# wells-wood-research/timed-design

Measured on AMD Instinct MI355X. Metric: residue_frames_per_sec, higher is better.
Workload: dtype f32

## Files before the change

timed-design_amd/csrc/common.h:

```cpp
#pragma once
#include <hip/hip_runtime.h>
#include <stdint.h>
#include <string>
#include <vector>

#include "../../include/timed_hip.h"

enum : int {
    OP_INPUT = 0, OP_CONV3D, OP_DENSE, OP_BN, OP_ACT, OP_MAXPOOL, OP_AVGPOOL, OP_GAP, OP_GMP,
    OP_FLATTEN, OP_CONCAT, OP_ADD, OP_IDENTITY
};
enum : int { ACT_LINEAR = 0, ACT_RELU, ACT_ELU, ACT_SOFTMAX, ACT_SIGMOID, ACT_TANH, ACT_LEAKY };

void th_set_error(const char* fmt, ...);
#define TH_FAIL(code, ...)          \
    do {                            \
        th_set_error(__VA_ARGS__);  \
        return (code);              \
    } while (0)
#define HIP_TRY(expr)                                                                            \
    do {                                                                                         \
        hipError_t _e = (expr);                                                                  \
        if (_e != hipSuccess) {                                                                  \
            th_set_error("%s failed: %s (%s:%d)", #expr, hipGetErrorString(_e), __FILE__, __LINE__); \
            return TH_EHIP;                                                                      \
        }                                                                                        \
    } while (0)

struct ThKnobs {
    int winograd = 1;
    int wino_split = 1;
    int wfused = 1;
    int wf_split = 1;
    int lanes = 1, lane_lag = 1;
    int guard = 1;
    int first_wino = 1;
    int first_split = 1;
    int conv_gl = 1;
    int dense_gemm = 1;
    int first_int = 1;
    int first_zb = 0;
    int first_dbg = 0;
    int no_pool_first = 0;
    int no_tail_fuse = 0;
    int conv_nogeo = 0, n16_nogeo = 0, conv_noxc = 0, conv_notail = 0, conv_nozmajor = 0, conv_nocompact = 0, conv_nopw = 0;
    int conv_bmode = 0;
    int conv_dbg = 0, conv_ldspad = 0, n16_resident = 0;
    int pw_nopipe = 0, pw_noepi = 0, pw_dbg = 0;
    int wf_resident = 0, wf_dbg = 0, wf_noblk = 0;
    long long wino_piece = 0;
    int wino_dbg = 0, wino_var = 3, wino_b3var = 0, wino_nomid = 0;
    std::string nondefault;
};
void th_knobs_read(ThKnobs* k);
inline const ThKnobs& th_knobs_of(const ThKnobs* k) { static const ThKnobs dflt; return k ? *k : dflt; }

hipError_t th_malloc_retry_impl(void** p, size_t bytes);
template <class T> inline hipError_t th_malloc_retry(T** p, size_t bytes) { return th_malloc_retry_impl(reinterpret_cast<void**>(p), bytes); }

int th_usable_cpus();

struct TView {
    float* p = nullptr;
    int D = 1, H = 1, W = 1, C = 0;
    int cs = 0;
    int coff = 0;
    int64_t fs = 0;
    int blk = 0;
    int V() const { return D * H * W; }
};

#define TH_MAX_POST 4
enum : int { POP_ACT = 1, POP_AFFINE = 2 };
struct PostOps {
    int n = 0;
    int type[TH_MAX_POST] = {0, 0, 0, 0};
    int act[TH_MAX_POST] = {0, 0, 0, 0};
    float alpha[TH_MAX_POST] = {0, 0, 0, 0};
    const float* scale[TH_MAX_POST] = {nullptr, nullptr, nullptr, nullptr};
    const float* shift[TH_MAX_POST] = {nullptr, nullptr, nullptr, nullptr};
    int monotone = 0;
};
struct PreOp {
    const float* scale = nullptr;
    const float* shift = nullptr;
    int act = ACT_LINEAR;
    float alpha = 0.f;
};

struct ConvGeom {
    int kd, kh, kw, sd, sh, sw, dd, dh, dw;
    int pz, py, px;
};
int launch_convert_frames(hipStream_t s, const void* src, int dtype, int64_t n, int V, int C, TView dst);
int launch_conv3d_direct(hipStream_t s, int64_t n, TView in, TView out, ConvGeom g, const float* w, const float* bias,
                         PreOp pre, PostOps post);
int launch_pool3d(hipStream_t s, int64_t n, TView in, TView out, ConvGeom g, int is_max);
int launch_eltwise(hipStream_t s, int64_t n, TView in, TView out, PostOps ops);
int launch_global_pool(hipStream_t s, int64_t n, TView in, TView out, int is_max);
int launch_dense(hipStream_t s, int64_t n, TView in, TView out, const float* w, const float* bias, PostOps post);
inline bool conv_gl_wanted(int knob, const ConvGeom& g, int Vo) { return knob == 2 || (knob == 1 && (g.sd > 1 || g.sh > 1 || g.sw > 1 || Vo <= 64)); }
bool conv_gl_ok(int Cin, int Cout, int in_cs, int in_coff, int64_t in_fs);
size_t conv_gl_wpk_floats(const ConvGeom& g, int Cin, int Cout);
double conv_gl_exec_flops(const ConvGeom& g, int Cin, int Cout, int Vo);
std::string conv_gl_label(int Cout);
void conv_gl_pack_weights(const ConvGeom& g, int Cin, int Cout, const float* w, float* dst);
int launch_conv_gl(hipStream_t s, int64_t n, TView in, TView out, ConvGeom g, int Cin, int Cout, const float* wpk, const float* bias, PreOp pre, PostOps post);
bool dense_gemm_ok(int F, int O, int64_t xfs);
int launch_dense_gemm(hipStream_t s, int64_t n, TView in, TView out, const float* w, const float* bias, PostOps post);
int launch_softmax(hipStream_t s, int64_t n, TView in, TView out);
int launch_gap_softmax(hipStream_t s, int64_t n, TView in, TView logits, TView probs);
int launch_tail_dense(hipStream_t s, int64_t n, TView in, PostOps pre, TView pooled, TView logits, TView probs, const float* w,
                      const float* bias, PostOps post, int softmax);
int launch_copy(hipStream_t s, int64_t n, TView in, TView out);
int launch_add(hipStream_t s, int64_t n, TView a, TView b, TView out);
int launch_synth_frames(hipStream_t s, float* d, int64_t n, int side, int channels, int atoms, uint64_t seed);

struct ConvMfmaPlan {
    int cfg = -1;
    int CI = 0, CS = 0;
    int BN = 0;
    int nnb = 0;
    int nchunks = 0;
    int pool = 0;
    int Dc = 0, Hc = 0, Wc = 0;
    int FB = 1, ZB = 0, nzb = 1;
    int Zp = 0, Hp = 0, Wp = 0;
    int rows_pf = 0;
    int bres = 0;
    int ncu = 0;
    size_t lds_bytes = 0;
    size_t tab_off = 0;
    size_t wpk_floats = 0;
    double exec_flops = 0;
    int first_wino = 0;
    double own_flops = 0;
    int geo = 0;
    const ThKnobs* knobs = nullptr;
    std::string label;
};
bool conv_mfma_plan(const TView& in, const TView& out_conv, const ConvGeom& g, int Cin, int Cout, int pool,
                    const ThKnobs& kn, ConvMfmaPlan* plan);
bool conv_mfma_plan_tail(const TView& in, const TView& out_conv, const ConvGeom& g, int Cin, int Cout, int pool,
                         const ConvMfmaPlan& main, const ThKnobs& kn, ConvMfmaPlan* tail, int* cout_main);
void conv_mfma_pack_weights(const ConvMfmaPlan& p, const ConvGeom& g, int Cin, int Cout, const float* w_keras,
                            float* dst);
int launch_conv_mfma(hipStream_t s, int64_t n, const ConvMfmaPlan& p, TView in, TView out, ConvGeom g, int Cin,
                     int Cout, const float* wpk, const float* bias, PreOp pre, PostOps post);

struct ConvWinoPlan {
    int P = 9;
    int Cin = 0, Cout = 0, Coutp = 0, ncb = 0;
    int Cinp = 0;
    size_t wpk_floats = 0;
    int64_t v_fpf = 0, m_fpf = 0;
    double gemm_flops = 0;
    double exec_flops = 0;
    int split = 0;
    int narrow = 0;
    const ThKnobs* knobs = nullptr;
    std::string label;
};
bool conv_wino_plan(const TView& in, const TView& out_conv, const ConvGeom& g, int Cin, int Cout, int scheme, int split, const ThKnobs& kn,
                    ConvWinoPlan* plan);
void conv_wino_pack_weights(const ConvWinoPlan& p, const float* w_keras, float* dst);
int launch_wino_in(hipStream_t s, int64_t n, const ConvWinoPlan& p, TView in, float* V, PreOp pre);
int launch_wino_gemm(hipStream_t s, int64_t n, const ConvWinoPlan& p, const float* V, float* M, const float* wpk);
int launch_wino_out(hipStream_t s, int64_t n, const ConvWinoPlan& p, const float* M, TView out, const float* bias, PostOps post, bool gap = false);
int launch_wino_mid(hipStream_t s, int64_t n, const ConvWinoPlan& p, const float* M, float* V_next, const float* bias, PostOps post);

struct ConvWfPlan {
    int geo = -1;
    int pool = 0;
    int Cin = 0, Cout = 0, ncb = 0, nchunks = 0;
    size_t wpk_floats = 0, lds_bytes = 0;
    double own_flops = 0;
    double exec_flops = 0;
    int ncu = 0;
    const ThKnobs* knobs = nullptr;
    std::string label;
};
bool conv_wf_plan(const TView& in, const TView& out_conv, const ConvGeom& g, int Cin, int Cout, int pool, const ThKnobs& kn, ConvWfPlan* plan);
bool conv_wf_view_ok(const TView& in);
int conv_wf_pre_kind(const PreOp& pre);
std::string conv_wf_label(const ConvWfPlan& p, const PreOp& pre);
void conv_wf_pack_weights(const ConvWfPlan& p, const float* w_keras, float* dst);
int launch_conv_wf(hipStream_t s, int64_t n, const ConvWfPlan& p, TView in, TView out, const float* wpk, const float* bias, PreOp pre,
                   PostOps post);

struct ConvWfsPlan {
    int geo = -1, pool = 0;
    int Cin = 0, Cout = 0, nkh = 0, ncp = 0;
    size_t wpk_floats = 0, lds_bytes = 0;
    double own_flops = 0, exec_flops = 0;
    int ncu = 0;
    const ThKnobs* knobs = nullptr;
    std::string label;
};
bool conv_wfs_plan(const ConvWfPlan& base, const TView& in, const PreOp& pre, const ThKnobs& kn, ConvWfsPlan* plan);
void conv_wfs_pack_weights(const ConvWfsPlan& p, const float* w_keras, float* dst);
int launch_conv_wfs(hipStream_t s, int64_t n, const ConvWfsPlan& p, TView in, TView out, const float* wpk, const float* bias, PostOps post);

int launch_sparse_expand(hipStream_t s, int64_t n, const uint32_t* bits, const uint64_t* vidx, const float* values, float* out, int E, int W);

std::string conv_first_label(const ConvMfmaPlan& p, int Cin, const PostOps& post);
bool conv_first_plan(int Din, int Hin, int Win, int Cin, const TView& out_conv, const ConvGeom& g, int Cout, int pool,
                     const ThKnobs& kn, ConvMfmaPlan* plan);
void conv_first_pack_weights(int Cin, int Cout, const float* w_keras, float* dst);
void conv_first_w_pack_weights(int Cin, int Cout, const float* w_keras, float* dst);
int launch_conv_first(hipStream_t s, int64_t n, const ConvMfmaPlan& p, const void* frames, int dtype, int Din, int Hin,
                      int Win, int Cin, TView out, ConvGeom g, int Cout, const float* wpk, const float* bias, PostOps post);
bool conv_first_b3_ok(const ConvMfmaPlan& p, int Din, int Hin, int Win, int Cin, int Cout, const ConvGeom& g, const PostOps& post);
size_t conv_first_b3_wpk_floats();
double conv_first_b3_exec_flops();
std::string conv_first_b3_label(int nnb);
void conv_first_b3_pack_weights(int Cin, int Cout, const float* w_keras, float* dst);
int launch_conv_first_b3(hipStream_t s, int64_t n, const ConvMfmaPlan& p, const void* frames, int dtype, int Cin, TView out, int Cout,
                         const float* wpk, const float* bias, PostOps post);

bool conv_first5_ok(int Din, int Hin, int Win, int Cin, int Cout, const ConvGeom& g, int pool, const ThKnobs& kn);
size_t conv_first5_wpk_floats();
double conv_first5_exec_flops();
std::string conv_first5_label();
void conv_first5_pack_weights(int Cin, int Cout, const float* w_keras, float* dst);
int launch_conv_first5(hipStream_t s, int64_t n, const ThKnobs* knobs, int ncu, const void* frames, int dtype, int Cin, TView out, int Cout,
                       const float* wpk, const float* bias, PostOps post);

bool conv_pw_plan(const TView& in, const TView& out_conv, const ConvGeom& g, int Cin, int Cout, int pool, const ThKnobs& kn, ConvMfmaPlan* plan);
void conv_pw_pack_weights(const ConvMfmaPlan& p, int Cin, int Cout, const float* w_keras, float* dst);
std::string conv_pw_label(const ConvMfmaPlan& p, bool out_blk, const PostOps& post);
int launch_conv_pw(hipStream_t s, int64_t n, const ConvMfmaPlan& p, TView in, TView out, int Cin, int Cout, const float* wpk,
                   const float* bias, PreOp pre, PostOps post);

int sampler_run(int device, const double* h_probs, int64_t n_res, int n_cls, int64_t n_samples, double temperature,
                int rng_mode, uint64_t seed, uint64_t rng_offset, const double* h_uniforms, int32_t* h_idx, double* h_r_out,
                const char* cat_letters, char* h_letters, double* h_q_out);
```

timed-design_amd/csrc/conv_wino.hip:

```cpp
#include "common.h"
#include "device_math.h"
#include "wino_tables.h"

#include <algorithm>
#include <cstdlib>
#include <cstring>
#include <thread>
#include <vector>

typedef float f32x16 __attribute__((ext_vector_type(16)));

namespace {

constexpr int kZ = WINO_N;
constexpr int kNF = 64;
constexpr int kKC = 32;
constexpr int kCB = 128;

template <int R, int C>
__device__ __forceinline__ void wino_apply(const float (&T)[R][C], const float (&in)[C], float (&out)[R]) {
#pragma unroll
    for (int r = 0; r < R; ++r) {
        float acc = 0.f;
        bool first = true;
// ... 318 lines not shown
                if (ph + 1 < kSlots * kZ) {
                    const int ns = (ph + 1) / kZ, nz = (ph + 1) % kZ;
                    af[cur ^ 1][0] = *reinterpret_cast<const float4*>(lds + aoff[ns] + (nz * kNF) * kKC);
                    af[cur ^ 1][1] = *reinterpret_cast<const float4*>(lds + aoff[ns] + (nz * kNF + 32) * kKC);
                }
                if (VAR == 1) __builtin_amdgcn_sched_barrier(0);
                const float av0[4] = {af[cur][0].x, af[cur][0].y, af[cur][0].z, af[cur][0].w};
                const float av1[4] = {af[cur][1].x, af[cur][1].y, af[cur][1].z, af[cur][1].w};
#pragma unroll
                for (int dz = 0; dz < 3; ++dz) {
                    if (!wino_tap_ok(zi, dz)) continue;
                    const int zo = zi - dz + 1;
                    const float4 b4 = bw[s & 1][dz];
                    const float bv[4] = {b4.x, b4.y, b4.z, b4.w};
#pragma unroll
                    for (int t = 0; t < 4; ++t) {
                        acc[zo][0] = __builtin_amdgcn_mfma_f32_32x32x2f32(av0[t], bv[t], acc[zo][0], 0, 0, 0);
                        acc[zo][1] = __builtin_amdgcn_mfma_f32_32x32x2f32(av1[t], bv[t], acc[zo][1], 0, 0, 0);
                    }
                }
                if (VAR == 1) __builtin_amdgcn_sched_barrier(0);
            }
        }
    }
    if (!active) return;
    float* mbase = a.M + ((int64_t)p * a.Ns + (int64_t)fb * kNF) * a.Coutp + cb * kCB + wave * 32 + j;
    const int64_t mz = (int64_t)a.npos * a.Ns * a.Coutp;
    if (a.dbg & 2) {
        float sum = 0.f;
#pragma unroll
        for (int z = 0; z < kZ; ++z)
#pragma unroll
            for (int rt = 0; rt < 2; ++rt)
#pragma unroll
                for (int r = 0; r < 16; ++r) sum += acc[z][rt][r];
        if (sum == 12345.678f) mbase[0] = sum;
        return;
    }
    if (VAR == 3) {
        __syncthreads();
        float* T = lds + wave * (32 * 36);
        const int rr = lane >> 3, c4 = (lane & 7) * 4;
        float* mb = a.M + ((int64_t)p * a.Ns + (int64_t)fb * kNF) * a.Coutp + cb * kCB + wave * 32 + c4;
#pragma unroll
        for (int z = 0; z < kZ; ++z)
#pragma unroll
            for (int rt = 0; rt < 2; ++rt) {
#pragma unroll
                for (int r = 0; r < 16; ++r) T[((r & 3) + 8 * (r >> 2) + 4 * h) * 36 + j] = acc[z][rt][r];
#pragma unroll
                for (int k = 0; k < 4; ++k) {
                    const int row = rr + 8 * k;
                    *reinterpret_cast<float4*>(mb + z * mz + (int64_t)(rt * 32 + row) * a.Coutp) = *reinterpret_cast<const float4*>(T + row * 36 + c4);
                }
            }
        return;
    }
#pragma unroll
    for (int z = 0; z < kZ; ++z)
#pragma unroll
        for (int rt = 0; rt < 2; ++rt)
#pragma unroll
            for (int r = 0; r < 16; ++r) {
                const int row = rt * 32 + (r & 3) + 8 * (r >> 2) + 4 * h;
                if (VAR == 2) __builtin_nontemporal_store(acc[z][rt][r], mbase + z * mz + (int64_t)row * a.Coutp);
                else mbase[z * mz + (int64_t)row * a.Coutp] = acc[z][rt][r];
            }
}


typedef __bf16 bf16x8 __attribute__((ext_vector_type(8)));
typedef __bf16 bf16x2 __attribute__((ext_vector_type(2)));
typedef float f32x2v __attribute__((ext_vector_type(2)));
typedef unsigned u32x4v __attribute__((ext_vector_type(4)));

__device__ __forceinline__ unsigned wino_pk_bf16(float lo, float hi) {
    return __builtin_bit_cast(unsigned, __builtin_convertvector((f32x2v){lo, hi}, bf16x2));
}
__device__ __forceinline__ float wino_bf16_lo(unsigned w) { return __builtin_bit_cast(float, w << 16); }
__device__ __forceinline__ float wino_bf16_hi(unsigned w) { return __builtin_bit_cast(float, w & 0xffff0000u); }

constexpr int kB3Slab = kZ * kNF * kKC * 2;

template <int VAR>
__global__ void __launch_bounds__(256, 2) k_wino_gemm_b3(const WinoGemmArgs a) {
    __shared__ __attribute__((aligned(16))) unsigned char lds[3 * kB3Slab];
    const unsigned xcd = blockIdx.x & 7u, slot = blockIdx.x >> 3;
    const unsigned L = xcd * a.per_xcd + slot;
    if (slot >= a.per_xcd || L >= a.total) return;
    const unsigned cb = L % (unsigned)a.ncb;
    const unsigned fb = (L / (unsigned)a.ncb) % (unsigned)a.nfb;
    const unsigned p = L / (unsigned)(a.ncb * a.nfb);
    const int tid = threadIdx.x, lane = tid & 63;
    const int wave = __builtin_amdgcn_readfirstlane(tid >> 6);
    const int j = lane & 31, h = lane >> 5;
    const int nchunks = a.Cin / kKC;
    const bool active = (int)(cb * kCB) + wave * 32 < a.Cout;
    const int S = nchunks * 6;
    const uint4* wq = reinterpret_cast<const uint4*>(a.U) + ((size_t)((p * a.ncb + cb) * 4 + wave) * S * 3) * 64 + lane;
    const float* vbase = a.V + ((int64_t)p * a.Ns + (int64_t)fb * kNF) * a.Cin;
    const int64_t zstride = (int64_t)a.npos * a.Ns * a.Cin;

    f32x16 acc[kZ][2];
#pragma unroll
    for (int z = 0; z < kZ; ++z)
#pragma unroll
        for (int rt = 0; rt < 2; ++rt)
#pragma unroll
            for (int r = 0; r < 16; ++r) acc[z][rt][r] = 0.f;

    uint4 bw[2][3];
#pragma unroll
    for (int pc = 0; pc < 3; ++pc) bw[0][pc] = wq[pc * 64];
    const int r0 = 8 * wave + (lane >> 3), g4 = lane & 7;
    __amdgpu_buffer_rsrc_t vrsrc[kZ];
#pragma unroll
    for (int z = 0; z < kZ; ++z) vrsrc[z] = __builtin_amdgcn_make_buffer_rsrc(const_cast<float*>(vbase + z * zstride), 0, 0xffffffffu, 0x00020000);
    const unsigned goff = (unsigned)(r0 * a.Cin + 4 * g4) * 4u;
    const unsigned rstride32_b = (unsigned)(32 * a.Cin * 4);
    unsigned char* const sdst = lds + r0 * 64 + (((g4 >> 1) ^ ((r0 >> 2) & 3)) << 4) + ((g4 & 1) << 3);
    const unsigned char* aptr[2];
#pragma unroll
    for (int ks = 0; ks < 2; ++ks) aptr[ks] = lds + j * 64 + (((2 * ks + h) ^ ((j >> 2) & 3)) << 4);

    for (int ch = 0; ch < nchunks; ++ch) {
        __syncthreads();
        {
            float4 x[10];
#pragma unroll
            for (int i = 0; i < 10; ++i)
                x[i] = (a.dbg & 1) ? make_float4(1.f, 2.f, 3.f, 4.f) :
                       __builtin_bit_cast(float4, __builtin_amdgcn_raw_buffer_load_b128(vrsrc[i >> 1], goff, (i & 1) * rstride32_b + ch * (kKC * 4), 0));
            __builtin_amdgcn_sched_barrier(0);
#pragma unroll
            for (int i = 0; i < 10; ++i) {
                const unsigned h01 = wino_pk_bf16(x[i].x, x[i].y), h23 = wino_pk_bf16(x[i].z, x[i].w);
                const float rx = x[i].x - wino_bf16_lo(h01), ry = x[i].y - wino_bf16_hi(h01);
                const float rz = x[i].z - wino_bf16_lo(h23), rw = x[i].w - wino_bf16_hi(h23);
                const unsigned m01 = wino_pk_bf16(rx, ry), m23 = wino_pk_bf16(rz, rw);
                const float sx = rx - wino_bf16_lo(m01), sy = ry - wino_bf16_hi(m01);
                const float sz = rz - wino_bf16_lo(m23), sw = rw - wino_bf16_hi(m23);
                const unsigned l01 = wino_pk_bf16(sx, sy), l23 = wino_pk_bf16(sz, sw);
                *reinterpret_cast<uint2*>(sdst + i * 2048) = make_uint2(h01, h23);
                *reinterpret_cast<uint2*>(sdst + i * 2048 + kB3Slab) = make_uint2(m01, m23);
                *reinterpret_cast<uint2*>(sdst + i * 2048 + 2 * kB3Slab) = make_uint2(l01, l23);
            }
        }
        __syncthreads();
        if (!active) continue;
#pragma unroll
        for (int st = 0; st < 6; ++st) {
            const int ks = st / 3, dz = st % 3, cur = st & 1;
            {
                const int sg = ch * 6 + st;
                const int nx = sg + 1 < S ? sg + 1 : sg;
                if (a.dbg & 4) {
#pragma unroll
                    for (int pc = 0; pc < 3; ++pc) bw[cur ^ 1][pc] = bw[cur][pc];
                } else
#pragma unroll
                for (int pc = 0; pc < 3; ++pc) bw[cur ^ 1][pc] = wq[(size_t)(nx * 3 + pc) * 64];
            }
            bf16x8 bf[3];
#pragma unroll
            for (int pc = 0; pc < 3; ++pc) bf[pc] = __builtin_bit_cast(bf16x8, bw[cur][pc]);
            const int nzi = 5 - (dz != 1), z0 = dz == 2 ? 1 : 0;
            bf16x8 af[2][2][3];
            auto read_a = [&](int set, int zi) {
#pragma unroll
// ... 100 lines not shown
        for (int q = 0; q < 4; ++q) {
            hw[q] = wino_pk_bf16(v[2 * q], v[2 * q + 1]);
            const float r0 = v[2 * q] - wino_bf16_lo(hw[q]), r1 = v[2 * q + 1] - wino_bf16_hi(hw[q]);
            mw[q] = wino_pk_bf16(r0, r1);
            const float s0 = r0 - wino_bf16_lo(mw[q]), s1 = r1 - wino_bf16_hi(mw[q]);
            lw[q] = wino_pk_bf16(s0, s1);
        }
        f[0] = __builtin_bit_cast(bf16x8, make_uint4(hw[0], hw[1], hw[2], hw[3]));
        f[1] = __builtin_bit_cast(bf16x8, make_uint4(mw[0], mw[1], mw[2], mw[3]));
        f[2] = __builtin_bit_cast(bf16x8, make_uint4(lw[0], lw[1], lw[2], lw[3]));
    };

    float4 xs[3][4];
    auto load_step = [&](float4 (&x)[4], int step_ch, int zi) {
        load_plane(x, step_ch < nchunks ? step_ch : nchunks - 1, zi);
    };
    load_step(xs[0], 0, 0);
    load_step(xs[1], 0, 1);
    for (int ch0 = 0; ch0 < nchunks; ch0 += 3) {
#pragma unroll
        for (int cc = 0; cc < 3; ++cc) {
            const int ch = ch0 + cc;
            if (ch >= nchunks) break;
            uint4 bw[2][3][3];
#pragma unroll
            for (int ks = 0; ks < 2; ++ks)
#pragma unroll
                for (int dz = 0; dz < 3; ++dz)
#pragma unroll
                    for (int pc = 0; pc < 3; ++pc) bw[ks][dz][pc] = wq[(size_t)(((ch * 2 + ks) * 3 + dz) * 3 + pc) * 64];
#pragma unroll
            for (int zi = 0; zi < kZ; ++zi) {
                const int t = cc * kZ + zi;
                float4 fr[4];
                transpose(xs[t % 3], fr);
                {
                    const int t2 = t + 2, c2 = ch0 + t2 / kZ, z2 = t2 % kZ;
                    load_step(xs[t2 % 3], c2, z2);
                }
                bf16x8 af[2][3];
                split8(fr[0], fr[1], af[0]);
                split8(fr[2], fr[3], af[1]);
                constexpr int PA[6] = {2, 0, 1, 1, 0, 0}, PB[6] = {0, 2, 1, 0, 1, 0};
#pragma unroll
                for (int q = 0; q < 6; ++q)
#pragma unroll
                    for (int ks = 0; ks < 2; ++ks)
#pragma unroll
                        for (int dz = 0; dz < 3; ++dz) {
                            if (!wino_tap_ok(zi, dz)) continue;
                            acc[zi - dz + 1] = __builtin_amdgcn_mfma_f32_32x32x16_bf16(af[ks][PA[q]], __builtin_bit_cast(bf16x8, bw[ks][dz][PB[q]]),
                                                                                       acc[zi - dz + 1], 0, 0, 0);
                        }
                __builtin_amdgcn_sched_barrier(0);
            }
        }
    }
    float* mb = a.M + ((int64_t)p * a.Ns + (int64_t)fb * 32) * a.Coutp + j;
    const int64_t mz = (int64_t)a.npos * a.Ns * a.Coutp;
#pragma unroll
    for (int z = 0; z < kZ; ++z)
#pragma unroll
        for (int r = 0; r < 16; ++r) mb[z * mz + (int64_t)((r & 3) + 8 * (r >> 2) + 4 * h) * a.Coutp] = acc[z][r];
}

}

bool conv_wino_plan(const TView& in, const TView& out, const ConvGeom& g, int Cin, int Cout, int scheme, int split, const ThKnobs& kn, ConvWinoPlan* p) {
    if (g.kd != 3 || g.kh != 3 || g.kw != 3 || g.sd != 1 || g.sh != 1 || g.sw != 1 || g.dd != 1 || g.dh != 1 || g.dw != 1) return false;
    if (g.pz != 1 || g.py != 1 || g.px != 1) return false;
    if (in.D != kZ || in.H != kZ || in.W != kZ || out.D != kZ || out.H != kZ || out.W != kZ) return false;
    const bool narrow = split && Cout <= 32 && Cin >= 128;
    if (Cin < kKC || (Cout < 64 && !narrow)) return false;
    if (scheme != 9 && scheme != 7) return false;
    const int kPos = scheme * scheme;
    p->P = scheme;
    p->Cin = Cin; p->Cout = Cout;
    p->Cinp = (Cin + kKC - 1) / kKC * kKC;
    const int Cinp = p->Cinp;
    p->narrow = narrow ? 1 : 0;
    p->Coutp = narrow ? 32 : (Cout + kCB - 1) / kCB * kCB;
    p->ncb = narrow ? 1 : p->Coutp / kCB;
    p->split = split ? 1 : 0;
    p->knobs = &kn;
    p->wpk_floats = (size_t)kPos * 3 * Cinp * p->Coutp * (p->split ? 3 : 2) / 2;
    p->v_fpf = (int64_t)kZ * kPos * Cinp;
    p->m_fpf = (int64_t)kZ * kPos * p->Coutp;
    p->gemm_flops = 2.0 * kPos * 13 * Cin * (double)Cout;
    p->exec_flops = 2.0 * kPos * 13 * Cinp * (double)((Cout + 31) / 32 * 32);
    p->label = std::string("conv_wino<") + (scheme == 9 ? "F(3,3)+F(2,3)" : "F(5,3)") + " in-plane, z direct; gemm " + (narrow ? "32f x 32" : "64f x " + std::to_string(kCB)) + "c, K" + std::to_string(Cinp) + (Cinp != Cin ? " (" + std::to_string(Cin) + " real)" : "") +
               (p->split ? "; bf16x3 split operands, 6 products, fp32 accumulate" : "") + ">";
    return true;
}

static inline uint16_t wino_bf16_rne(float f) {
    uint32_t u;
    std::memcpy(&u, &f, 4);
    if ((u & 0x7f800000u) == 0x7f800000u) return (uint16_t)(u >> 16);
    u += 0x7fffu + ((u >> 16) & 1u);
    return (uint16_t)(u >> 16);
}
static inline double wino_bf16_val(uint16_t b) {
    const uint32_t u = (uint32_t)b << 16;
    float f;
    std::memcpy(&f, &u, 4);
    return (double)f;
}
static inline void wino_split3(double x, uint16_t (&pc)[3]) {
    pc[0] = wino_bf16_rne((float)x);
    const double r1 = x - wino_bf16_val(pc[0]);
    pc[1] = wino_bf16_rne((float)r1);
    const double r2 = r1 - wino_bf16_val(pc[1]);
    pc[2] = wino_bf16_rne((float)r2);
}

void conv_wino_pack_weights(const ConvWinoPlan& p, const float* w, float* dst) {
    const int Cin = p.Cin, Cinp = p.Cinp, Cout = p.Cout, S = Cinp / 8, ncb = p.ncb, kP = p.P;
    auto G = [kP](int a, int j) { return kP == 9 ? kWinoG9[a][j] : kWinoG7[a][j]; };
    std::memset(dst, 0, p.wpk_floats * sizeof(float));
    auto work = [&](int ci_lo, int ci_hi) {
        std::vector<double> t((size_t)kP * 3 * Cout), u((size_t)Cout);
        for (int ci = ci_lo; ci < ci_hi; ++ci) {
            const int s = ci / 8, hh = (ci % 8) / 4, tt = ci % 4;
            for (int dz = 0; dz < 3; ++dz) {
                for (int a = 0; a < kP; ++a)
                    for (int k = 0; k < 3; ++k) {
                        double* tr = &t[((size_t)a * 3 + k) * Cout];
                        std::fill(tr, tr + Cout, 0.0);
                        for (int jj = 0; jj < 3; ++jj) {
                            const double g = G(a, jj);
                            if (g == 0.0) continue;
                            const float* wr = w + ((((size_t)dz * 3 + jj) * 3 + k) * Cin + ci) * Cout;
                            for (int co = 0; co < Cout; ++co) tr[co] += g * (double)wr[co];
                        }
                    }
                for (int a = 0; a < kP; ++a)
                    for (int b = 0; b < kP; ++b) {
                        std::fill(u.begin(), u.end(), 0.0);
                        for (int k = 0; k < 3; ++k) {
                            const double g = G(b, k);
                            if (g == 0.0) continue;
                            const double* tr = &t[((size_t)a * 3 + k) * Cout];
                            for (int co = 0; co < Cout; ++co) u[co] += g * tr[co];
                        }
                        const int pos = a * kP + b;
                        if (p.narrow) {
                            uint16_t* d16 = reinterpret_cast<uint16_t*>(dst);
                            const int chunk = ci / kKC, h16 = (ci % kKC) / 16, ks = (ci % 16) / 8, e = ci % 8, nch = Cinp / kKC;
                            for (int co = 0; co < Cout; ++co) {
                                uint16_t pc[3];
                                wino_split3(u[co], pc);
                                const size_t frag = ((size_t)(pos * nch + chunk) * 2 + ks) * 3 + dz;
                                for (int q = 0; q < 3; ++q) d16[((frag * 3 + q) * 64 + (h16 * 32 + co)) * 8 + e] = pc[q];
                            }
                            continue;
                        }
                        if (p.split) {
                            uint16_t* d16 = reinterpret_cast<uint16_t*>(dst);
                            const int chunk = ci / kKC, ks = (ci % kKC) / 16, h8 = (ci % 16) / 8, e = ci % 8, nsteps = (Cinp / kKC) * 6;
                            for (int co = 0; co < Cout; ++co) {
                                const int cb = co / kCB, wv = (co % kCB) / 32, j = co % 32;
                                uint16_t pc[3];
                                wino_split3(u[co], pc);
                                const size_t step = (size_t)((pos * ncb + cb) * 4 + wv) * nsteps + (size_t)(chunk * 2 + ks) * 3 + dz;
                                for (int q = 0; q < 3; ++q) d16[((step * 3 + q) * 64 + (h8 * 32 + j)) * 8 + e] = pc[q];
                            }
                            continue;
                        }
                        for (int co = 0; co < Cout; ++co) {
                            const int cb = co / kCB, wv = (co % kCB) / 32, j = co % 32;
                            dst[((((size_t)(pos * ncb + cb) * 4 + wv) * S + s) * 3 + dz) * 256 + (hh * 32 + j) * 4 + tt] = (float)u[co];
                        }
                    }
            }
        }
    };
    const int nt = std::max(1, std::min({th_usable_cpus(), 32, Cin / 8}));
    if (nt == 1) { work(0, Cin); return; }
    std::vector<std::thread> th;
    for (int k = 0; k < nt; ++k) th.emplace_back(work, (int)((int64_t)Cin * k / nt), (int)((int64_t)Cin * (k + 1) / nt));
    for (auto& x : th) x.join();
}

static int64_t wino_piece(const ConvWinoPlan& p, int64_t n, int64_t Ns, int64_t fs, int width) {
    const int64_t lim = (1ll << 31) - 1;
    if (Ns * width > lim) return 0;
    const int64_t forced = th_knobs_of(p.knobs).wino_piece;
    const int64_t piece = std::max<int64_t>(1, std::min<int64_t>(n, lim / std::max<int64_t>(fs, 1)));
    return forced > 0 ? std::min(piece, forced) : piece;
}

int launch_wino_in(hipStream_t s, int64_t n, const ConvWinoPlan& p, TView in, float* V, PreOp pre) {
    if (n <= 0) return TH_OK;
    const int64_t Ns = (n + kNF - 1) / kNF * kNF;
    const int64_t piece = wino_piece(p, n, Ns, in.fs, p.Cinp);
    if (!piece) TH_FAIL(TH_EUNSUP, "conv_wino: %lld frames per launch exceed the 32-bit offsets of the transform kernels", (long long)n);
    const bool has_pre = pre.scale || pre.act != ACT_LINEAR;
    for (int64_t f0 = 0; f0 < n; f0 += piece) {
        const int64_t cnt = std::min(piece, n - f0);
        WinoInArgs ia;
        ia.in = in.p + f0 * in.fs; ia.in_fs = in.fs; ia.in_cs = in.cs; ia.in_coff = in.coff; ia.Cin = p.Cinp; ia.Creal = p.Cin; ia.pre = pre;
        ia.V = V + f0 * p.Cinp; ia.Ns = Ns; ia.n = cnt;
        const dim3 grid((unsigned)((cnt * p.Cinp + 255) / 256));
        if (p.P == 9) {
            if (has_pre) hipLaunchKernelGGL((k_wino_in<true, 9>), grid, dim3(256), 0, s, ia);
            else hipLaunchKernelGGL((k_wino_in<false, 9>), grid, dim3(256), 0, s, ia);
        } else {
            if (has_pre) hipLaunchKernelGGL((k_wino_in<true, 7>), grid, dim3(256), 0, s, ia);
            else hipLaunchKernelGGL((k_wino_in<false, 7>), grid, dim3(256), 0, s, ia);
        }
    }
    HIP_TRY(hipGetLastError());
    return TH_OK;
}

int launch_wino_gemm(hipStream_t s, int64_t n, const ConvWinoPlan& p, const float* V, float* M, const float* wpk) {
    if (n <= 0) return TH_OK;
    WinoGemmArgs ga;
    ga.V = V; ga.U = wpk; ga.M = M; ga.Ns = (n + kNF - 1) / kNF * kNF; ga.Cin = p.Cinp; ga.Coutp = p.Coutp;
    ga.Cout = p.Cout;
    ga.nfb = (int)(ga.Ns / kNF); ga.ncb = p.ncb;
    ga.npos = p.P * p.P;
    ga.total = (unsigned)(ga.npos * ga.nfb * ga.ncb);
    ga.per_xcd = (ga.total + 7) / 8;
    const ThKnobs& kn = th_knobs_of(p.knobs);
    ga.dbg = kn.wino_dbg;
    const int var = kn.wino_var;
    if (p.narrow) {
        const int64_t groups = (ga.Ns / 32 + 3) / 4;
        hipLaunchKernelGGL(k_wino_gemm_n32, dim3((unsigned)(ga.npos * groups)), dim3(256), 0, s, ga);
    } else if (p.split) {
        const int bvar = kn.wino_b3var;
        if (bvar == 1) hipLaunchKernelGGL(k_wino_gemm_b3<1>, dim3(ga.per_xcd * 8), dim3(256), 0, s, ga);
        else hipLaunchKernelGGL(k_wino_gemm_b3<0>, dim3(ga.per_xcd * 8), dim3(256), 0, s, ga);
    }
    else if (var == 0) hipLaunchKernelGGL(k_wino_gemm<0>, dim3(ga.per_xcd * 8), dim3(256), 0, s, ga);
    else if (var == 2) hipLaunchKernelGGL(k_wino_gemm<2>, dim3(ga.per_xcd * 8), dim3(256), 0, s, ga);
    else if (var == 3) hipLaunchKernelGGL(k_wino_gemm<3>, dim3(ga.per_xcd * 8), dim3(256), 0, s, ga);
    else hipLaunchKernelGGL(k_wino_gemm<1>, dim3(ga.per_xcd * 8), dim3(256), 0, s, ga);
    HIP_TRY(hipGetLastError());
    return TH_OK;
}

int launch_wino_out(hipStream_t s, int64_t n, const ConvWinoPlan& p, const float* M, TView out, const float* bias, PostOps post, bool gap) {
    if (n <= 0) return TH_OK;
    const int64_t Ns = (n + kNF - 1) / kNF * kNF;
    const int64_t piece = wino_piece(p, n, Ns, out.fs, p.Coutp);
    if (!piece) TH_FAIL(TH_EUNSUP, "conv_wino: %lld frames per launch exceed the 32-bit offsets of the transform kernels", (long long)n);
    for (int64_t f0 = 0; f0 < n; f0 += piece) {
        const int64_t cnt = std::min(piece, n - f0);
        WinoOutArgs oa;
        oa.M = M + f0 * p.Coutp; oa.Ns = Ns; oa.Coutp = p.Coutp; oa.Cout = p.Cout; oa.bias = bias; oa.post = post;
        oa.out = out.p + f0 * out.fs; oa.out_fs = out.fs; oa.out_cs = out.cs; oa.out_coff = out.coff; oa.n = cnt;
        const dim3 grid((unsigned)((cnt * p.Cout + 255) / 256));
        if (gap) {
            if (p.P == 9) hipLaunchKernelGGL((k_wino_out<9, true>), grid, dim3(256), 0, s, oa);
            else hipLaunchKernelGGL((k_wino_out<7, true>), grid, dim3(256), 0, s, oa);
        } else if (p.P == 9) hipLaunchKernelGGL(k_wino_out<9>, grid, dim3(256), 0, s, oa);
        else hipLaunchKernelGGL(k_wino_out<7>, grid, dim3(256), 0, s, oa);
    }
    HIP_TRY(hipGetLastError());
    return TH_OK;
}

int launch_wino_mid(hipStream_t s, int64_t n, const ConvWinoPlan& p, const float* M, float* V_next, const float* bias, PostOps post) {
    if (n <= 0) return TH_OK;
    const int64_t Ns = (n + kNF - 1) / kNF * kNF;
    if (Ns * (int64_t)p.Coutp >= (1ll << 31))
        TH_FAIL(TH_EUNSUP, "conv_wino: %lld frames per launch exceed the 32-bit offsets of the transform kernels", (long long)n);
    const int Cn = (p.Cout + kKC - 1) / kKC * kKC;
    if (Ns * (int64_t)Cn >= (1ll << 31))
        TH_FAIL(TH_EUNSUP, "conv_wino: %lld frames per launch exceed the 32-bit offsets of the transform kernels", (long long)n);
    WinoMidArgs ma;
    ma.M = M; ma.Ns = Ns; ma.Coutp = p.Coutp; ma.C = p.Cout; ma.Cn = Cn; ma.bias = bias; ma.post = post; ma.V = V_next; ma.n = n;
    const dim3 grid((unsigned)((n * (int64_t)Cn + 255) / 256));
    if (p.P == 9) hipLaunchKernelGGL(k_wino_mid<9>, grid, dim3(256), 0, s, ma);
    else hipLaunchKernelGGL(k_wino_mid<7>, grid, dim3(256), 0, s, ma);
    HIP_TRY(hipGetLastError());
    return TH_OK;
}
```

timed-design_amd/csrc/runtime.hip:

```cpp
#include "common.h"

#include <algorithm>
#include <chrono>
#include <cmath>
#include <cstdarg>
#include <cstdio>
#include <cstring>
#include <functional>
#include <map>
#include <memory>
#include <mutex>
#include <set>

#include <dlfcn.h>
#include <sys/stat.h>
#include <unistd.h>

static thread_local char g_err[1024] = "";
void th_set_error(const char* fmt, ...) {
    va_list ap;
    va_start(ap, fmt);
    vsnprintf(g_err, sizeof g_err, fmt, ap);
    va_end(ap);
}

void th_knobs_read(ThKnobs* k) {
    *k = ThKnobs();
    std::string& nd = k->nondefault;
    auto note = [&](const char* name, const char* v) { nd += (nd.empty() ? "" : " "); nd += name; nd += "="; nd += v; };
    auto num = [&](const char* name, int* dst, int lo, int hi) {
        const char* e = getenv(name);
        if (!e) return;
        const int v = std::max(lo, std::min(hi, atoi(e)));
        if (v != *dst) note(name, e);
        *dst = v;
    };
    auto flag = [&](const char* name, int* dst) {
        const char* e = getenv(name);
        if (e && *e && atoi(e) != 0) { *dst = 1; note(name, e); }
    };
    num("TH_WINOGRAD", &k->winograd, 0, 2);
    num("TH_WINO_SPLIT", &k->wino_split, 0, 1);
    num("TH_WFUSED", &k->wfused, 0, 1);
    num("TH_WF_SPLIT", &k->wf_split, 0, 1);
    if (const char* e = getenv("TH_LANES")) { k->lanes = atoi(e) == 2 ? 2 : 1; if (k->lanes != 1) note("TH_LANES", e); }
    num("TH_LANE_LAG", &k->lane_lag, 0, 1 << 20);
    num("TH_GUARD", &k->guard, 0, 2);
    num("TH_FIRST_WINO", &k->first_wino, 0, 1);
    num("TH_FIRST_SPLIT", &k->first_split, 0, 1);
    num("TH_FIRST_INT", &k->first_int, 0, 1);
    num("TH_DENSE_GEMM", &k->dense_gemm, 0, 1);
    num("TH_CONV_GL", &k->conv_gl, 0, 2);
    num("TH_FIRST_ZB", &k->first_zb, 0, 1 << 20);
    num("TH_FIRST_DBG", &k->first_dbg, 0, 1 << 20);
    flag("TH_NO_POOL_FIRST", &k->no_pool_first);
    flag("TH_NO_TAIL_FUSE", &k->no_tail_fuse);
    flag("TH_CONV_NOGEO", &k->conv_nogeo);
    flag("TH_N16_NOGEO", &k->n16_nogeo);
    flag("TH_CONV_NOXC", &k->conv_noxc);
    flag("TH_CONV_NOTAIL", &k->conv_notail);
    flag("TH_CONV_NOZMAJOR", &k->conv_nozmajor);
    flag("TH_CONV_NOCOMPACT", &k->conv_nocompact);
    flag("TH_CONV_NOPW", &k->conv_nopw);
    if (const char* e = getenv("TH_CONV_BMODE")) {
        k->conv_bmode = !std::strcmp(e, "dbuf") ? 1 : !std::strcmp(e, "stream8") ? 2 : !std::strcmp(e, "no16") ? 3 : 0;
        if (k->conv_bmode) note("TH_CONV_BMODE", e);
    }
    num("TH_CONV_DBG", &k->conv_dbg, 0, 1 << 20);
    num("TH_CONV_LDSPAD", &k->conv_ldspad, 0, 160 * 1024);
    num("TH_N16_RESIDENT", &k->n16_resident, 0, 1 << 20);
    flag("TH_PW_NOPIPE", &k->pw_nopipe);
    flag("TH_PW_NOEPI", &k->pw_noepi);
    num("TH_PW_DBG", &k->pw_dbg, 0, 1 << 20);
    num("TH_WF_RESIDENT", &k->wf_resident, 0, 1 << 20);
    num("TH_WF_DBG", &k->wf_dbg, 0, 1 << 20);
    num("TH_WF_NOBLK", &k->wf_noblk, 0, 1);
    if (const char* e = getenv("TH_WINO_PIECE")) { k->wino_piece = std::max(0ll, atoll(e)); if (k->wino_piece) note("TH_WINO_PIECE", e); }
    num("TH_WINO_DBG", &k->wino_dbg, 0, 1 << 20);
    num("TH_WINO_VAR", &k->wino_var, 0, 3);
    num("TH_WINO_B3VAR", &k->wino_b3var, 0, 1);
    num("TH_WINO_NOMID", &k->wino_nomid, 0, 1);
}

namespace {
struct DevCache {
    std::mutex mu;
    struct Blk { void* p; uint64_t stamp; };
    std::multimap<std::pair<int, size_t>, Blk> free_blocks;
    std::map<void*, std::pair<int, size_t>> live;
    std::map<int, size_t> cached_bytes;
    std::map<int, size_t> cap_bytes;
    uint64_t clock = 0;
    static constexpr size_t kCacheBytes = 24ull << 30;
    static constexpr size_t kCacheBlocks = 1024;
};
DevCache g_cache;

size_t cache_cap_locked(int device) {
    auto it = g_cache.cap_bytes.find(device);
    if (it != g_cache.cap_bytes.end()) return it->second;
    size_t cap = DevCache::kCacheBytes, free_b = 0, total_b = 0;
    int cur = -1;
    if (hipGetDevice(&cur) == hipSuccess && (cur == device || hipSetDevice(device) == hipSuccess)) {
        if (hipMemGetInfo(&free_b, &total_b) == hipSuccess && total_b) cap = std::min(cap, total_b / 8);
        if (cur >= 0 && cur != device) (void)hipSetDevice(cur);
    }
    (void)hipGetLastError();
    g_cache.cap_bytes[device] = cap;
    return cap;
}

int cached_malloc(void** out, size_t bytes, int device) {
    if (!bytes) bytes = 4;
    {
        std::lock_guard<std::mutex> lock(g_cache.mu);
        auto it = g_cache.free_blocks.find({device, bytes});
        if (it != g_cache.free_blocks.end()) {
            *out = it->second.p;
            g_cache.free_blocks.erase(it);
            g_cache.cached_bytes[device] -= bytes;
            g_cache.live[*out] = {device, bytes};
            return TH_OK;
        }
    }
    hipError_t e = th_malloc_retry(out, bytes);
    if (e != hipSuccess) {
        (void)hipGetLastError();
        TH_FAIL(e == hipErrorOutOfMemory ? TH_ENOMEM : TH_EHIP, "hipMalloc(%zu) failed: %s", bytes, hipGetErrorString(e));
    }
    std::lock_guard<std::mutex> lock(g_cache.mu);
    g_cache.live[*out] = {device, bytes};
    return TH_OK;
}

void cached_free(void* p) {
    if (!p) return;
    std::vector<void*> evict;
    {
        std::lock_guard<std::mutex> lock(g_cache.mu);
        auto it = g_cache.live.find(p);
        if (it == g_cache.live.end()) { (void)hipFree(p); return; }
        const std::pair<int, size_t> key = it->second;
        g_cache.live.erase(it);
        const size_t cap = cache_cap_locked(key.first);
        if (key.second > cap) evict.push_back(p);
        else {
            g_cache.free_blocks.insert({key, {p, ++g_cache.clock}});
            g_cache.cached_bytes[key.first] += key.second;
            while (g_cache.cached_bytes[key.first] > cap || g_cache.free_blocks.size() > DevCache::kCacheBlocks) {
                auto oldest = g_cache.free_blocks.end();
                for (auto b = g_cache.free_blocks.begin(); b != g_cache.free_blocks.end(); ++b)
                    if ((b->first.first == key.first || g_cache.free_blocks.size() > DevCache::kCacheBlocks) &&
                        (oldest == g_cache.free_blocks.end() || b->second.stamp < oldest->second.stamp))
                        oldest = b;
                if (oldest == g_cache.free_blocks.end()) break;
                evict.push_back(oldest->second.p);
                g_cache.cached_bytes[oldest->first.first] -= oldest->first.second;
                g_cache.free_blocks.erase(oldest);
            }
        }
    }
    for (void* q : evict) (void)hipFree(q);
}
// ... 2029 lines not shown
```

Before: 584,700.

## Add 16x16x32 bf16 MFMA variant of split-precision Winograd GEMM and default to it

Adds a new b3 Winograd GEMM variant that uses 16x16x32 bf16 MFMA tiles instead of the 32-wide ones, with a swizzled LDS layout for the three-way bf16-split activations, buffer-resource loads, and a matching weight packing order. It is made the default for split-precision, non-narrow layers. The intent is better MFMA throughput and fewer LDS bank conflicts in the split-bf16 emulated-fp32 GEMM. In exchange it uses more accumulator registers and a new weight layout, and it adds an LDS-staged epilogue.

Result: faster. 631,300 (median of 6 runs) (+8.0%).

```diff
diff --git a/timed-design_amd/csrc/common.h b/timed-design_amd/csrc/common.h
--- a/timed-design_amd/csrc/common.h
+++ b/timed-design_amd/csrc/common.h
@@ -49,7 +49,7 @@
     int pw_nopipe = 0, pw_noepi = 0, pw_dbg = 0;
     int wf_resident = 0, wf_dbg = 0, wf_noblk = 0;
     long long wino_piece = 0;
-    int wino_dbg = 0, wino_var = 3, wino_b3var = 0, wino_nomid = 0;
+    int wino_dbg = 0, wino_var = 3, wino_b3var = 2, wino_nomid = 0;
     std::string nondefault;
 };
 void th_knobs_read(ThKnobs* k);
@@ -158,6 +158,7 @@
     double exec_flops = 0;
     int split = 0;
     int narrow = 0;
+    int b3var = 0;
     const ThKnobs* knobs = nullptr;
     std::string label;
 };
diff --git a/timed-design_amd/csrc/conv_wino.hip b/timed-design_amd/csrc/conv_wino.hip
--- a/timed-design_amd/csrc/conv_wino.hip
+++ b/timed-design_amd/csrc/conv_wino.hip
@@ -424,9 +424,155 @@
 
 constexpr int kB3Slab = kZ * kNF * kKC * 2;
 
+__device__ __forceinline__ constexpr int wino_b3_sw16(int R) { return ((R >> 2) & 3) ^ (((R >> 2) & 1) << 1); }
+
+typedef float f32x4 __attribute__((ext_vector_type(4)));
+
+__device__ __forceinline__ void wino_gemm_b3_16(const WinoGemmArgs& a, unsigned char* lds) {
+    const unsigned xcd = blockIdx.x & 7u, slot = blockIdx.x >> 3;
+    const unsigned L = xcd * a.per_xcd + slot;
+    if (slot >= a.per_xcd || L >= a.total) return;
+    const unsigned cb = L % (unsigned)a.ncb;
+    const unsigned fb = (L / (unsigned)a.ncb) % (unsigned)a.nfb;
+    const unsigned p = L / (unsigned)(a.ncb * a.nfb);
+    const int tid = threadIdx.x, lane = tid & 63;
+    const int wave = __builtin_amdgcn_readfirstlane(tid >> 6);
+    const int r16 = lane & 15, g16 = lane >> 4;
+    const int nchunks = a.Cin / kKC;
+    const bool active = (int)(cb * kCB) + wave * 32 < a.Cout;
+    const __amdgpu_buffer_rsrc_t wrsrc = __builtin_amdgcn_make_buffer_rsrc(
+        const_cast<float*>(a.U + ((size_t)((p * a.ncb + cb) * 4 + wave) * nchunks * 18) * 256), 0, 0xffffffffu, 0x00020000);
+    const unsigned woff = (unsigned)lane * 16u;
+    const float* vbase = a.V + ((int64_t)p * a.Ns + (int64_t)fb * kNF) * a.Cin;
+    const int64_t zstride = (int64_t)a.npos * a.Ns * a.Cin;
+
+    f32x4 acc[kZ][4][2];
+#pragma unroll
+    for (int z = 0; z < kZ; ++z)
+#pragma unroll
+        for (int rt = 0; rt < 4; ++rt)
+#pragma unroll
+            for (int ct = 0; ct < 2; ++ct) acc[z][rt][ct] = (f32x4){0.f, 0.f, 0.f, 0.f};
+
+    const int r0 = 8 * wave + (lane >> 3), g4 = lane & 7;
+    __amdgpu_buffer_rsrc_t vrsrc[kZ];
+#pragma unroll
+    for (int z = 0; z < kZ; ++z) vrsrc[z] = __builtin_amdgcn_make_buffer_rsrc(const_cast<float*>(vbase + z * zstride), 0, 0xffffffffu, 0x00020000);
+    const unsigned goff = (unsigned)(r0 * a.Cin + 4 * g4) * 4u;
+    const unsigned rstride32_b = (unsigned)(32 * a.Cin * 4);
+    unsigned char* const sdst = lds + r0 * 64 + (((g4 >> 1) ^ wino_b3_sw16(r0)) << 4) + ((g4 & 1) << 3);
+    const unsigned char* const aptr = lds + r16 * 64 + ((g16 ^ wino_b3_sw16(r16)) << 4);
+
+    uint4 bw[2][3][3];
+    auto load_b = [&](int ch, int ct) {
+        if (a.dbg & 4) {
+            const unsigned k = woff ^ ((unsigned)(ch * 2 + ct) << 4);
+#pragma unroll
+            for (int dz = 0; dz < 3; ++dz)
+#pragma unroll
+                for (int pc = 0; pc < 3; ++pc)
+                    bw[ct][dz][pc] = make_uint4(0x3f813f82u ^ (k << (dz + pc)), 0x3e833e84u ^ k, 0x3d853d86u + (k << pc), 0x3c873c88u ^ (k << dz));
+            return;
+        }
+#pragma unroll
+        for (int dz = 0; dz < 3; ++dz)
+#pragma unroll
+            for (int pc = 0; pc < 3; ++pc)
+                bw[ct][dz][pc] = __builtin_bit_cast(uint4, __builtin_amdgcn_raw_buffer_load_b128(wrsrc, woff, (((ch * 2 + ct) * 3 + dz) * 3 + pc) * 1024, 0));
+    };
+
+    for (int ch = 0; ch < nchunks; ++ch) {
+        __syncthreads();
+        {
+            float4 x[10];
+#pragma unroll
+            for (int i = 0; i < 10; ++i)
+                x[i] = (a.dbg & 1) ? make_float4(1.f, 2.f, 3.f, 4.f) :
+                       __builtin_bit_cast(float4, __builtin_amdgcn_raw_buffer_load_b128(vrsrc[i >> 1], goff, (i & 1) * rstride32_b + ch * (kKC * 4), 0));
+            __builtin_amdgcn_sched_barrier(0);
+#pragma unroll
+            for (int i = 0; i < 10; ++i) {
+                const unsigned h01 = wino_pk_bf16(x[i].x, x[i].y), h23 = wino_pk_bf16(x[i].z, x[i].w);
+                const float rx = x[i].x - wino_bf16_lo(h01), ry = x[i].y - wino_bf16_hi(h01);
+                const float rz = x[i].z - wino_bf16_lo(h23), rw = x[i].w - wino_bf16_hi(h23);
+                const unsigned m01 = wino_pk_bf16(rx, ry), m23 = wino_pk_bf16(rz, rw);
+                const float sx = rx - wino_bf16_lo(m01), sy = ry - wino_bf16_hi(m01);
+                const float sz = rz - wino_bf16_lo(m23), sw = rw - wino_bf16_hi(m23);
+                const unsigned l01 = wino_pk_bf16(sx, sy), l23 = wino_pk_bf16(sz, sw);
+                *reinterpret_cast<uint2*>(sdst + i * 2048) = make_uint2(h01, h23);
+                *reinterpret_cast<uint2*>(sdst + i * 2048 + kB3Slab) = make_uint2(m01, m23);
+                *reinterpret_cast<uint2*>(sdst + i * 2048 + 2 * kB3Slab) = make_uint2(l01, l23);
+            }
+        }
+        load_b(ch, 0);
+        load_b(ch, 1);
+        __syncthreads();
+        if (!active) continue;
+#pragma unroll
+        for (int zi = 0; zi < kZ; ++zi)
+#pragma unroll
+            for (int rt = 0; rt < 4; ++rt) {
+                bf16x8 af[3];
+#pragma unroll
+                for (int pc = 0; pc < 3; ++pc)
+                    af[pc] = __builtin_bit_cast(bf16x8, *reinterpret_cast<const uint4*>(aptr + pc * kB3Slab + (zi * kNF + rt * 16) * 64));
+#pragma unroll
+                for (int dz = 0; dz < 3; ++dz) {
+                    if (!wino_tap_ok(zi, dz)) continue;
+                    const int zo = zi - dz + 1;
+                    constexpr int PA[6] = {2, 0, 1, 1, 0, 0}, PB[6] = {0, 2, 1, 0, 1, 0};
+#pragma unroll
+                    for (int c = 0; c < 6; ++c)
+#pragma unroll
+                        for (int ct = 0; ct < 2; ++ct)
+                            acc[zo][rt][ct] = __builtin_amdgcn_mfma_f32_16x16x32_bf16(af[PA[c]], __builtin_bit_cast(bf16x8, bw[ct][dz][PB[c]]),
+                                                                                     acc[zo][rt][ct], 0, 0, 0);
+                }
+                __builtin_amdgcn_sched_barrier(0);
+            }
+    }
+    if (!active) return;
+    if (a.dbg & 2) {
+        float sum = 0.f;
+#pragma unroll
+        for (int z = 0; z < kZ; ++z)
+#pragma unroll
+            for (int rt = 0; rt < 4; ++rt)
+#pragma unroll
+                for (int ct = 0; ct < 2; ++ct)
+#pragma unroll
+                    for (int r = 0; r < 4; ++r) sum += acc[z][rt][ct][r];
+        if (sum == 12345.678f) a.M[0] = sum;
+        return;
+    }
+    __syncthreads();
+    float* T = reinterpret_cast<float*>(lds) + wave * (16 * 36);
+    const int rr = lane >> 3, c4 = (lane & 7) * 4;
+    float* mb = a.M + ((int64_t)p * a.Ns + (int64_t)fb * kNF) * a.Coutp + cb * kCB + wave * 32 + c4;
+    const int64_t mz = (int64_t)a.npos * a.Ns * a.Coutp;
+#pragma unroll
+    for (int z = 0; z < kZ; ++z)
+#pragma unroll
+        for (int rt = 0; rt < 4; ++rt) {
+#pragma unroll
+            for (int ct = 0; ct < 2; ++ct)
+#pragma unroll
+                for (int r = 0; r < 4; ++r) T[(4 * g16 + r) * 36 + ct * 16 + r16] = acc[z][rt][ct][r];
+#pragma unroll
+            for (int k = 0; k < 2; ++k) {
+                const int row = rr + 8 * k;
+                *reinterpret_cast<float4*>(mb + z * mz + (int64_t)(rt * 16 + row) * a.Coutp) = *reinterpret_cast<const float4*>(T + row * 36 + c4);
+            }
+        }
+}
+
 template <int VAR>
 __global__ void __launch_bounds__(256, 2) k_wino_gemm_b3(const WinoGemmArgs a) {
     __shared__ __attribute__((aligned(16))) unsigned char lds[3 * kB3Slab];
+    if constexpr (VAR == 2) {
+        wino_gemm_b3_16(a, lds);
+        return;
+    }
     const unsigned xcd = blockIdx.x & 7u, slot = blockIdx.x >> 3;
     const unsigned L = xcd * a.per_xcd + slot;
     if (slot >= a.per_xcd || L >= a.total) return;
@@ -693,6 +839,7 @@
     p->Coutp = narrow ? 32 : (Cout + kCB - 1) / kCB * kCB;
     p->ncb = narrow ? 1 : p->Coutp / kCB;
     p->split = split ? 1 : 0;
+    p->b3var = split && !narrow ? kn.wino_b3var : 0;
     p->knobs = &kn;
     p->wpk_floats = (size_t)kPos * 3 * Cinp * p->Coutp * (p->split ? 3 : 2) / 2;
     p->v_fpf = (int64_t)kZ * kPos * Cinp;
@@ -766,6 +913,18 @@
                             }
                             continue;
                         }
+                        if (p.split && p.b3var == 2) {
+                            uint16_t* d16 = reinterpret_cast<uint16_t*>(dst);
+                            const int chunk = ci / kKC, g8 = (ci % kKC) / 8, e = ci % 8, nch = Cinp / kKC;
+                            for (int co = 0; co < Cout; ++co) {
+                                const int cb = co / kCB, wv = (co % kCB) / 32, ct = (co % 32) / 16, c = co % 16;
+                                uint16_t pc[3];
+                                wino_split3(u[co], pc);
+                                const size_t frag = ((size_t)(((pos * ncb + cb) * 4 + wv) * nch + chunk) * 2 + ct) * 3 + dz;
+                                for (int q = 0; q < 3; ++q) d16[((frag * 3 + q) * 64 + (g8 * 16 + c)) * 8 + e] = pc[q];
+                            }
+                            continue;
+                        }
                         if (p.split) {
                             uint16_t* d16 = reinterpret_cast<uint16_t*>(dst);
                             const int chunk = ci / kKC, ks = (ci % kKC) / 16, h8 = (ci % 16) / 8, e = ci % 8, nsteps = (Cinp / kKC) * 6;
@@ -841,8 +1000,9 @@
         const int64_t groups = (ga.Ns / 32 + 3) / 4;
         hipLaunchKernelGGL(k_wino_gemm_n32, dim3((unsigned)(ga.npos * groups)), dim3(256), 0, s, ga);
     } else if (p.split) {
-        const int bvar = kn.wino_b3var;
-        if (bvar == 1) hipLaunchKernelGGL(k_wino_gemm_b3<1>, dim3(ga.per_xcd * 8), dim3(256), 0, s, ga);
+        const int bvar = p.b3var;
+        if (bvar == 2) hipLaunchKernelGGL(k_wino_gemm_b3<2>, dim3(ga.per_xcd * 8), dim3(256), 0, s, ga);
+        else if (bvar == 1) hipLaunchKernelGGL(k_wino_gemm_b3<1>, dim3(ga.per_xcd * 8), dim3(256), 0, s, ga);
         else hipLaunchKernelGGL(k_wino_gemm_b3<0>, dim3(ga.per_xcd * 8), dim3(256), 0, s, ga);
     }
     else if (var == 0) hipLaunchKernelGGL(k_wino_gemm<0>, dim3(ga.per_xcd * 8), dim3(256), 0, s, ga);
diff --git a/timed-design_amd/csrc/runtime.hip b/timed-design_amd/csrc/runtime.hip
--- a/timed-design_amd/csrc/runtime.hip
+++ b/timed-design_amd/csrc/runtime.hip
@@ -78,7 +78,7 @@
     if (const char* e = getenv("TH_WINO_PIECE")) { k->wino_piece = std::max(0ll, atoll(e)); if (k->wino_piece) note("TH_WINO_PIECE", e); }
     num("TH_WINO_DBG", &k->wino_dbg, 0, 1 << 20);
     num("TH_WINO_VAR", &k->wino_var, 0, 3);
-    num("TH_WINO_B3VAR", &k->wino_b3var, 0, 1);
+    num("TH_WINO_B3VAR", &k->wino_b3var, 0, 2);
     num("TH_WINO_NOMID", &k->wino_nomid, 0, 1);
 }
 
```
